# rajabala/Volumetric-Particles-For-Unity

Hardware: AMD Instinct MI355X
Metric: Mvoxels/s filled + Msamples/s raymarched, 32³×32³ grid @1080p (higher is better)
Workload: dtype f32 compute / f16 voxel storage

## Files before the change

### volumetric-particles-for-unity_amd/csrc/api.cpp

```cpp
#include <cmath>
#include <cstdarg>
#include <cstdio>
#include <cstdlib>
#include <cstring>
#include <new>

#include "vpfx_internal.h"

thread_local std::string g_vp_create_error;

int vp_fail(vp_ctx* c, int code, const char* fmt, ...)
{
    char buf[512];
    va_list ap;
    va_start(ap, fmt);
    vsnprintf(buf, sizeof buf, fmt, ap);
    va_end(ap);
    if (c) c->err = buf; else g_vp_create_error = buf;
    return code;
}

namespace {

template <typename T>
// ... 184 lines not shown

VP_EXPORT int vp_abi_version(void) { return VPFX_ABI_VERSION; }

VP_EXPORT const char* vp_last_error(const vp_ctx* c) { return c ? c->err.c_str() : g_vp_create_error.c_str(); }

VP_EXPORT int vp_create(const vp_config* cfg, vp_ctx** out)
{
    if (!cfg || !out) return vp_fail(nullptr, VP_ERR_BAD_ARG, "vp_create: null argument");
    *out = nullptr;
    if (cfg->num_devices < 0 || cfg->num_devices > VP_MAX_LOCAL_DEVICES || cfg->world_size < 0 || cfg->world_size > VP_MAX_RANKS)
        return vp_fail(nullptr, VP_ERR_BAD_ARG, "vp_create: num_devices %d / world_size %d out of range", cfg->num_devices, cfg->world_size);
    if (cfg->num_devices > 1 || cfg->world_size > 1 || (cfg->multi_flags & VP_MULTI_FORCE)) return multi_create(cfg, out);
    if (cfg->num_devices == 1) {
        vp_config one = *cfg;
        one.device = cfg->devices[0];
        return vp_create_single(&one, out);
    }
    return vp_create_single(cfg, out);
}

int vp_create_single(const vp_config* cfg, vp_ctx** out)
{
    vp_ctx* c = nullptr;
    *out = nullptr;
    const int nv = cfg->num_voxels;
    if (cfg->num_mv[0] < 1 || cfg->num_mv[1] < 1 || cfg->num_mv[2] < 1 || !(cfg->mv_scale > 0.f) || cfg->num_border < 0 ||
        2 * cfg->num_border >= nv || cfg->width < 1 || cfg->height < 1)
        return vp_fail(nullptr, VP_ERR_BAD_ARG, "vp_create: bad grid/screen configuration");
    if (nv < 2 || nv > 64)
        return vp_fail(nullptr, VP_ERR_UNSUPPORTED, "vp_create: num_voxels %d outside [2, 64]", nv);
    if ((cfg->reserved[0] != 0 && cfg->reserved[0] != 1) || (cfg->reserved[1] != 0 && cfg->reserved[1] != 1) || cfg->reserved[2] != 0)
        return vp_fail(nullptr, VP_ERR_BAD_ARG, "vp_create: vp_config.reserved = {%d, %d, %d} (0 or the documented switches; an uninitialised struct?)",
                       cfg->reserved[0], cfg->reserved[1], cfg->reserved[2]);
    if ((size_t)cfg->num_mv[0] * cfg->num_mv[1] * cfg->num_mv[2] > ((size_t)1 << 28))
        return vp_fail(nullptr, VP_ERR_UNSUPPORTED, "vp_create: grid too large");
    int z0 = cfg->slab_z0, z1 = cfg->slab_z1;
    if (z0 == 0 && z1 == 0) z1 = cfg->num_mv[2];
    if (z0 < 0 || z1 > cfg->num_mv[2] || z0 >= z1) return vp_fail(nullptr, VP_ERR_BAD_ARG, "vp_create: bad slab [%d,%d)", z0, z1);

    int ndev = 0;
    hipError_t e = hipGetDeviceCount(&ndev);
    if (e != hipSuccess || ndev < 1)
        return vp_fail(nullptr, VP_ERR_NO_DEVICE, "vp_create: no HIP device (%s); libvpfx has no CPU fallback",
                       e != hipSuccess ? hipGetErrorString(e) : "device count 0");
    int dev = cfg->device;
    if (dev < 0) { if (hipGetDevice(&dev) != hipSuccess) dev = 0; }
    if (dev >= ndev) return vp_fail(nullptr, VP_ERR_BAD_ARG, "vp_create: device %d of %d", dev, ndev);

    c = new (std::nothrow) vp_ctx();
    if (!c) return vp_fail(nullptr, VP_ERR_OOM, "vp_create: host allocation failed");
    c->cfg = *cfg;
    c->device = dev;
    if (cfg->multi_flags & VP_MULTI_TEST_HOOKS) { const char* hook = getenv("VPFX_TEST_CHAIN_TIMEOUT"); c->test_chain_timeout = hook && hook[0] == '1'; }
#if VPFX_AB
    { const char* sw = getenv("VPFX_NO_ZPROFILE"); c->no_zprofile = sw && sw[0] == '1'; }
    { const char* sw = getenv("VPFX_RM_FLAT"); c->rm_flat = sw && sw[0] == '1'; }
    { const char* sw = getenv("VPFX_RM_XCD_AFFINE"); c->rm_xcd_affine = sw && sw[0] == '1'; }
#endif
    c->n3 = (size_t)cfg->num_mv[0] * cfg->num_mv[1] * cfg->num_mv[2];
    memset(c->L, 0, sizeof c->L); c->L[0] = c->L[5] = c->L[10] = c->L[15] = 1.f;
    c->h_mvPos = (float*)malloc(c->n3 * 3 * sizeof(float));
    int rc = VP_OK;
    auto fail = [&](int code) { g_vp_create_error = c->err; vp_destroy_single(c); return code; };
    if (!c->h_mvPos) { c->err = "vp_create: host allocation failed"; return fail(VP_ERR_OOM); }
    hl_build_grid(c);
    if ((rc = ensure_device(c))) return fail(rc);
    if (hipDeviceGetAttribute(&c->num_cus, hipDeviceAttributeMultiprocessorCount, dev) != hipSuccess || c->num_cus < 1) c->num_cus = 256;
    const size_t nxy = (size_t)cfg->num_mv[0] * cfg->num_mv[1];
    if ((rc = dev_alloc(c, &c->d_mvPos, c->n3 * 3)) || (rc = dev_alloc(c, &c->d_count, c->n3)) ||
        (rc = dev_alloc(c, &c->d_offsets, c->n3 + 1)) || (rc = dev_alloc(c, &c->d_cursor, c->n3)) ||
        (rc = dev_alloc(c, &c->d_brick_index, c->n3)) || (rc = dev_alloc(c, &c->d_occ_list, c->n3)) ||
        (rc = dev_alloc(c, &c->d_onecol, 2)) || (rc = dev_alloc(c, &c->d_work_counter, 1)) || (rc = dev_alloc(c, &c->d_meta, 1)) ||
        (rc = dev_alloc(c, &c->d_ord, c->n3)) || (rc = dev_alloc(c, &c->d_colcount, nxy)) || (rc = dev_alloc(c, &c->d_chain, lightmap_elems(c))) ||
        (rc = dev_alloc(c, (int4**)&c->d_scan_totals, (c->n3 + 1023) / 1024 + 1)) ||
        (rc = dev_alloc(c, &c->d_lightmap, lightmap_elems(c))) || (rc = dev_alloc(c, &c->d_rank, nxy)) ||
        (rc = dev_alloc(c, &c->d_image, image_elems(c))) || (rc = dev_alloc(c, &c->d_samples, 1)) ||
        (rc = dev_alloc(c, &c->d_zsamples, (size_t)VPFX_ZPROF_COPIES * cfg->num_mv[2])) ||
        (rc = dev_alloc(c, &c->d_tile_order, (size_t)rm_order_ints(rm_num_super_tiles(cfg->width, cfg->height)) + rm_num_super_tiles(cfg->width, cfg->height) + 8)))
        return fail(rc);
#if VPFX_AB
    {
        const int sgx = rm_super_tiles_x(cfg->width), sgy = rm_super_tiles_y(cfg->height), ns = sgx * sgy;
        int side = 1; while (side < sgx || side < sgy) side <<= 1;
        std::vector<int> curve; curve.reserve(ns);
        for (long long d = 0; d < (long long)side * side; ++d) {
            long long tt = d; int x = 0, y = 0;
            for (int sdim = 1; sdim < side; sdim <<= 1) {
                const int rx = 1 & (int)(tt / 2), ry = 1 & ((int)tt ^ rx);
                if (ry == 0) { if (rx == 1) { x = sdim - 1 - x; y = sdim - 1 - y; } const int tmp = x; x = y; y = tmp; }
                x += sdim * rx; y += sdim * ry; tt /= 4;
            }
            if (x < sgx && y < sgy) curve.push_back(y * sgx + x);
        }
        if ((int)curve.size() == ns && (rc = dev_alloc(c, &c->d_tile_curve, (size_t)ns)) == VP_OK) {
            if (hipMemcpy(c->d_tile_curve, curve.data(), (size_t)ns * sizeof(int), hipMemcpyHostToDevice) != hipSuccess) { c->err = "hipMemcpy failed"; return fail(VP_ERR_HIP); }
        } else if (rc) return fail(rc);
    }
#endif
    if (hipHostMalloc((void**)&c->h_meta_host, 2 * sizeof(DevMeta), hipHostMallocMapped | hipHostMallocCoherent) != hipSuccess ||
        hipHostGetDevicePointer((void**)&c->d_meta_host, c->h_meta_host, 0) != hipSuccess) { c->err = "hipHostMalloc failed"; return fail(VP_ERR_HIP); }
    c->h_meta_host[0] = c->h_meta_host[1] = DevMeta{};
    if (hipHostMalloc((void**)&c->h_chain_err, sizeof(int), hipHostMallocMapped) != hipSuccess ||
        hipHostGetDevicePointer((void**)&c->d_chain_err, c->h_chain_err, 0) != hipSuccess) { c->err = "hipHostMalloc failed"; return fail(VP_ERR_HIP); }
    *c->h_chain_err = 0;
    if (hipMemset(c->d_chain, 0, lightmap_elems(c) * sizeof(unsigned long long)) != hipSuccess) { c->err = "hipMemset failed"; return fail(VP_ERR_HIP); }
    for (int s = 0; s < 4; ++s)
        for (int j = 0; j < 2; ++j)
            if (hipEventCreate(&c->ev[s][j]) != hipSuccess) { c->err = "hipEventCreate failed"; return fail(VP_ERR_HIP); }
    *out = c;
    return VP_OK;
}

VP_EXPORT void vp_destroy(vp_ctx* c)
{
    if (!c) return;
    if (c->multi) { multi_destroy(c); return; }
    vp_destroy_single(c);
}

void vp_destroy_single(vp_ctx* c)
{
    if (!c) return;
    (void)hipSetDevice(c->device);
    if (c->stream) (void)hipStreamSynchronize(c->stream); else (void)hipDeviceSynchronize();
    void* dev[] = {c->d_mvPos, c->d_raw, c->d_ws, c->d_rec, c->d_count, c->d_offsets, c->d_cursor, c->d_brick_index,
                   c->d_occ_list, c->d_ids_tmp, c->d_ids, c->d_onecol, c->d_work_counter, c->d_ord, c->d_colcount, c->d_chain, c->d_cube_u8, c->d_meta, c->d_scan_totals, c->d_bricks, c->d_dens_ao,
                   c->d_lightmap, c->d_cubequads, c->d_depthmap, c->d_occluders, c->d_mvtrans, c->d_brick_hit, c->d_rank, c->d_tile_order, c->d_tile_curve, c->d_image, c->d_scene_depth, c->d_samples, c->d_zsamples, c->d_cellinfo, c->d_occmask};
    for (void* p : dev) if (p) (void)hipFree(p);
    mesh_free_all(c);
    device_emitters_orphan_all(c);
    particle_queries_free(c);
    if (c->h_chain_err) (void)hipHostFree(c->h_chain_err);
    if (c->h_meta_host) (void)hipHostFree(c->h_meta_host);
    if (c->copy_stream) { (void)hipStreamSynchronize(c->copy_stream); (void)hipStreamDestroy(c->copy_stream); }
    if (c->ev_image_ready) (void)hipEventDestroy(c->ev_image_ready);
    if (c->ev_image_copied) (void)hipEventDestroy(c->ev_image_copied);
    for (int s = 0; s < 4; ++s) for (int j = 0; j < 2; ++j) if (c->ev[s][j]) (void)hipEventDestroy(c->ev[s][j]);
    free(c->h_mvPos);
    delete c;
}

VP_EXPORT int vp_pin_host_buffer(vp_ctx* c, void* ptr, uint64_t bytes)
{
    if (!c) return VP_ERR_BAD_ARG;
    if (!ptr || !bytes) return vp_fail(c, VP_ERR_BAD_ARG, "vp_pin_host_buffer: null buffer");
    if (c->multi) { VP_HIP(hipHostRegister(ptr, (size_t)bytes, hipHostRegisterPortable)); return VP_OK; }
    int rc = ensure_device(c); if (rc) return rc;
    VP_HIP(hipHostRegister(ptr, (size_t)bytes, hipHostRegisterDefault));
    return VP_OK;
}

VP_EXPORT int vp_unpin_host_buffer(vp_ctx* c, void* ptr)
{
    if (!c) return VP_ERR_BAD_ARG;
    if (!ptr) return vp_fail(c, VP_ERR_BAD_ARG, "vp_unpin_host_buffer: null buffer");
    if (c->multi) { int rcm = multi_sync(c); if (rcm) return rcm; VP_HIP(hipHostUnregister(ptr)); return VP_OK; }
    int rc = ensure_device(c); if (rc) return rc;
    if (c->stream) (void)hipStreamSynchronize(c->stream); else (void)hipDeviceSynchronize();
    if (c->image_copy_pending) { VP_HIP(hipEventSynchronize(c->ev_image_copied)); c->image_copy_pending = false; }
    VP_HIP(hipHostUnregister(ptr));
    return VP_OK;
}

VP_EXPORT int vp_set_stream(vp_ctx* c, void* hip_stream)
{
    if (!c) return VP_ERR_BAD_ARG;
    VP_NO_FANOUT(c, "vp_set_stream (a fan-out context owns one stream per device)");
    c->stream = (hipStream_t)hip_stream;
    return VP_OK;
}

VP_EXPORT int vp_sync(vp_ctx* c)
{
    if (!c) return VP_ERR_BAD_ARG;
    if (c->multi) return multi_sync(c);
    int rc = ensure_device(c); if (rc) return rc;
    { int rcs = stream_sync(c); if (rcs) return rcs; }
    if (c->image_copy_pending) { VP_HIP(hipEventSynchronize(c->ev_image_copied)); c->image_copy_pending = false; }
    return VP_OK;
}
// ... 774 lines not shown
```

### volumetric-particles-for-unity_amd/csrc/raymarch.hip

```cpp
#define VPFX_RM_MAIN_TU 1
#include "raymarch_kernels.h"

namespace {

__device__ __forceinline__ void tile_cost(const RmConsts& k, const int* __restrict__ brick_index, int sgx, float* __restrict__ cost_out, const int sti)
{
    __shared__ float part[4];
    const int wave = threadIdx.x >> 6, lane = threadIdx.x & 63;
    constexpr int SW = 16 << VPFX_RM_LX, SH = 16 << VPFX_RM_LY;
    const float colf = fminf((float)((sti % sgx) * SW + SW / 4 + (SW / 2) * (wave & 1)), (float)k.W - 1.f);
    const float rowf = fminf((float)((sti / sgx) * SH + SH / 4 + (SH / 2) * (wave >> 1)), (float)k.H - 1.f);
    float dx = (2.0f * (colf + 0.5f) / (float)k.W) - 1.0f;
    const float dy = (2.0f * (rowf + 0.5f) / (float)k.H) - 1.0f;
    dx *= k.aspect;
    const float dz = k.neg_inv_tan;
    const float inv = 1.0f / sqrtf((dx * dx + dy * dy) + dz * dz);
    const float dir[3] = {dx * inv, dy * inv, dz * inv};
    const float st = k.zMin / dir[2];
    float o[3], d[3];
#pragma unroll
    for (int r = 0; r < 3; ++r) {
        d[r] = (k.c2g[4 * r] * dir[0] + k.c2g[4 * r + 1] * dir[1]) + k.c2g[4 * r + 2] * dir[2];
        o[r] = d[r] * st + k.c2g[4 * r + 3];
    }
// ... 14 lines not shown
        const int gx = (int)floorf(fmaf(t, d[0], o[0])), gy = (int)floorf(fmaf(t, d[1], o[1])), gz = (int)floorf(fmaf(t, d[2], o[2]));
        const bool occ = gx >= 0 && gx < k.Nx && gy >= 0 && gy < k.Ny && gz >= k.z0 && gz < k.z1 &&
                         brick_index[(gz * k.Ny + gy) * k.Nx + gx] >= 0;
        c = (float)__popcll(__ballot(occ)) * (t1 - t0);
    }
    if (lane == 0) part[wave] = c;
    __syncthreads();
    if (threadIdx.x == 0) cost_out[sti] = (part[0] + part[1]) + (part[2] + part[3]);
}

#define RM_RANK_LDS 4096
#define RM_RANK_COLS 16
__device__ __forceinline__ void column_rank(const RmConsts& k, const float* __restrict__ mvPos, int* __restrict__ rank_out, const int blk)
{
    __shared__ __attribute__((aligned(16))) float keys[RM_RANK_LDS];
    __shared__ int partial[RM_RANK_COLS];
    const int nxy = k.Nx * k.Ny;
    auto key_of = [&](int j) -> float {
        const float dx = mvPos[3 * j] - k.cam_world[0], dy = mvPos[3 * j + 1] - k.cam_world[1], dz = mvPos[3 * j + 2] - k.cam_world[2];
        return (dx * dx + dy * dy) + dz * dz;
    };
    const int i = blk * RM_RANK_COLS + ((int)threadIdx.x & (RM_RANK_COLS - 1)), chunk = (int)threadIdx.x / RM_RANK_COLS;
    if (nxy > RM_RANK_LDS) {
        if (chunk == 0 && i < nxy) {
            const float ki = key_of(i);
            int r = 0;
            for (int j = 0; j < nxy; ++j) { const float kj = key_of(j); r += (kj < ki || (kj == ki && j < i)) ? 1 : 0; }
            rank_out[i] = r;
        }
        return;
    }
    const int npad = (nxy + 3) & ~3;
    for (int j = threadIdx.x; j < npad; j += 256) keys[j] = j < nxy ? key_of(j) : 3.0e38f;
    if (threadIdx.x < RM_RANK_COLS) partial[threadIdx.x] = 0;
    __syncthreads();
    if (i < nxy) {
        constexpr int NCHUNK = 256 / RM_RANK_COLS;
        const int per = ((npad + 4 * NCHUNK - 1) / (4 * NCHUNK)) * 4, j0 = chunk * per, j1 = min(npad, j0 + per);
        const float ki = keys[i];
        int r = 0;
        for (int j = j0; j < j1; j += 4) {
            const float4 kj = *reinterpret_cast<const float4*>(&keys[j]);
            r += (kj.x < ki || (kj.x == ki && j < i)) ? 1 : 0;
            r += (kj.y < ki || (kj.y == ki && j + 1 < i)) ? 1 : 0;
            r += (kj.z < ki || (kj.z == ki && j + 2 < i)) ? 1 : 0;
            r += (kj.w < ki || (kj.w == ki && j + 3 < i)) ? 1 : 0;
        }
        atomicAdd(&partial[threadIdx.x & (RM_RANK_COLS - 1)], r);
    }
    __syncthreads();
    if (chunk == 0 && i < nxy) rank_out[i] = partial[threadIdx.x];
}

__global__ void __launch_bounds__(256)
k_rm_prepare(RmConsts k, const int* __restrict__ brick_index, const float* __restrict__ mvPos, int n3, float4* __restrict__ mvtrans,
             float4* __restrict__ cellinfo , uint32_t* __restrict__ occmask , int* __restrict__ brick_hit,
             unsigned long long* __restrict__ samples, int nprep, int sgx, float* __restrict__ cost_out, int ncost, int* __restrict__ rank_out)
{
    if ((int)blockIdx.x >= nprep + ncost) { column_rank(k, mvPos, rank_out, (int)blockIdx.x - nprep - ncost); return; }
    if ((int)blockIdx.x >= nprep) { tile_cost(k, brick_index, sgx, cost_out, (int)blockIdx.x - nprep); return; }
    const int mi = blockIdx.x * 256 + threadIdx.x;
    if (mi == 0) *samples = 0ull;
    if (mi >= n3) return;
    const int slot = brick_index[mi];
    if (slot >= 0) {
        const float mx = mvPos[3 * mi], my = mvPos[3 * mi + 1], mz = mvPos[3 * mi + 2];
        float tr[3];
#pragma unroll
        for (int r = 0; r < 3; ++r) {
            const float a = k.inv_rows[r * 3], b = k.inv_rows[r * 3 + 1], c = k.inv_rows[r * 3 + 2];
            const float t = -((a * mx + b * my) + c * mz);
            tr[r] = ((a * k.c2w_t[0] + b * k.c2w_t[1]) + c * k.c2w_t[2]) + t * k.c2w_t[3];
        }
        mvtrans[slot] = make_float4(tr[0], tr[1], tr[2], 0.f);
        if (cellinfo) cellinfo[mi] = make_float4(tr[0], tr[1], tr[2], __int_as_float(slot));
        brick_hit[slot] = 0;
    } else if (cellinfo) {
        const float e = __int_as_float(-1);
        cellinfo[mi] = make_float4(e, e, e, e);
    }
    if (occmask && mi % k.Nx == 0) {
        uint32_t word = 0;
        for (int x = 0; x < k.Nx; ++x) word |= (brick_index[mi + x] >= 0 ? 1u : 0u) << x;
        occmask[mi / k.Nx] = word;
    }
}

__global__ void __launch_bounds__(256)
k_order_index(RmConsts k, const int* __restrict__ occ_list, const int* __restrict__ brick_index, const int* __restrict__ rank, int n,
              float4* __restrict__ mvtrans)
{
    const int i = blockIdx.x * 256 + threadIdx.x;
    if (i >= n) return;
    const int nxy = k.Nx * k.Ny, mi = occ_list[i], zz = mi / nxy, cell = mi % nxy;
    const int* occ = brick_index + zz * nxy;
    const int r = rank[cell];
    const bool phaseA = zz <= k.zB;
    int before_in_slice = 0, lower_cells = 0;
    for (int j = 0; j < nxy; ++j) {
        if (occ[j] < 0) continue;
        lower_cells += j < cell ? 1 : 0;
        before_in_slice += (phaseA ? rank[j] > r : rank[j] < r) ? 1 : 0;
    }
    mvtrans[i].w = __int_as_float((i - lower_cells) + before_in_slice);
}

#define MAX_PARTIALS 32
struct BlendArgs { const float4* img[MAX_PARTIALS]; int kind[MAX_PARTIALS]; int n; };

__global__ void __launch_bounds__(256)
k_blend(BlendArgs a, size_t npix, float4* __restrict__ out)
{
    const size_t i = (size_t)blockIdx.x * 256 + threadIdx.x;
    if (i >= npix) return;
    float4 d = make_float4(0.f, 0.f, 0.f, 0.f);
    for (int j = 0; j < a.n; ++j) {
        const float4 s = a.img[j][i];
        if (a.kind[j] == 0) { const float ia = 1.0f - s.w; d.x = s.x + d.x * ia; d.y = s.y + d.y * ia; d.z = s.z + d.z * ia; d.w = s.w + d.w * ia; }
        else { const float ia = 1.0f - d.w; d.x = s.x * ia + d.x; d.y = s.y * ia + d.y; d.z = s.z * ia + d.z; d.w = s.w * ia + d.w; }
    }
    out[i] = d;
}

__global__ void __launch_bounds__(256)
k_composite(const float4* __restrict__ particles, float4* __restrict__ scene, size_t npix)
{
    const size_t i = (size_t)blockIdx.x * 256 + threadIdx.x;
    if (i >= npix) return;
    const float4 s = particles[i];
    float4 d = scene[i];
    const float ia = 1.0f - s.w;
    d.x = s.x + d.x * ia; d.y = s.y + d.y * ia; d.z = s.z + d.z * ia; d.w = s.w + d.w;
    scene[i] = d;
}

}

int launch_raymarch(vp_ctx* c, const RmConsts& k_in, float* d_over, float* d_under, const RmHandoff* handoff)
{
    RmConsts k = k_in;
    k.occ_lds = (VPFX_RM_OCC_LDS && VPFX_RM_CELLINFO && k.Nx <= 32 && k.Nz * k.Ny <= VPFX_RM_OCC_WORDS) ? 1 : 0;
    const RmHandoff ho = (handoff && d_under) ? *handoff : RmHandoff{};
    const int early_out = (c->cfg.no_early_out == 1 || (k.flags & (VP_RM_NO_EARLY_OUT | VP_RM_SHOW_NUM_SAMPLES | VP_RM_SHOW_BLEND_FUNC | VP_RM_SHOW_DRAW_ORDER))) ? 0 : 1;
    k.flags &= ~VP_RM_NO_EARLY_OUT;
    const int nocc = c->h_meta.occupied;
    if ((size_t)nocc > c->mvtrans_cap) {
        if (c->d_mvtrans) VP_HIP(hipFree(c->d_mvtrans));
        c->d_mvtrans = nullptr; c->mvtrans_cap = 0;
        VP_HIP(hipMalloc((void**)&c->d_mvtrans, ((size_t)nocc + nocc / 8 + 16) * sizeof(float4)));
        c->mvtrans_cap = (size_t)nocc + nocc / 8 + 16;
    }
    if ((size_t)nocc > c->brick_hit_cap) {
        if (c->d_brick_hit) VP_HIP(hipFree(c->d_brick_hit));
        c->d_brick_hit = nullptr; c->brick_hit_cap = 0;
        VP_HIP(hipMalloc((void**)&c->d_brick_hit, ((size_t)nocc + nocc / 8 + 16) * sizeof(int)));
        c->brick_hit_cap = (size_t)nocc + nocc / 8 + 16;
    }
#if VPFX_RM_CELLINFO
    if (!c->d_cellinfo) VP_HIP(hipMalloc((void**)&c->d_cellinfo, c->n3 * sizeof(float4)));
    if (k.occ_lds && !c->d_occmask) VP_HIP(hipMalloc((void**)&c->d_occmask, VPFX_RM_OCC_WORDS * sizeof(uint32_t)));
#endif
    c->brick_hit_n = nocc;
    VP_HIP(hipEventRecord(c->ev[2][0], c->stream));
    {
        const int nprep = (int)((c->n3 + 255) / 256), nsuper = rm_num_super_tiles(k.W, k.H);
        const bool ordered = rm_ordered(c, k);
        float* cost = reinterpret_cast<float*>(c->d_tile_order + rm_order_ints(nsuper));
        const int ncost = ordered ? nsuper : 0, nrank = (k.Nx * k.Ny + RM_RANK_COLS - 1) / RM_RANK_COLS;
        hipLaunchKernelGGL(k_rm_prepare, dim3((unsigned)(nprep + ncost + nrank)), dim3(256), 0, c->stream, k, c->d_brick_index, c->d_mvPos,
                           (int)c->n3, c->d_mvtrans, c->d_cellinfo, k.occ_lds ? c->d_occmask : (uint32_t*)nullptr, c->d_brick_hit, c->d_samples,
                           nprep, rm_super_tiles_x(k.W), cost, ncost, c->d_rank);
    }
    if (nocc > 0) {
        if (k.flags & VP_RM_SHOW_DRAW_ORDER)
            hipLaunchKernelGGL(k_order_index, dim3((nocc + 255) / 256), dim3(256), 0, c->stream, k, c->d_occ_list, c->d_brick_index, c->d_rank,
                               nocc, c->d_mvtrans);
    }
    switch (k.nv) {
    case 16: launch_rm_nv<16>(c, k, d_over, d_under, early_out, ho); break;
    case 32: launch_rm_nv<32>(c, k, d_over, d_under, early_out, ho); break;
    case 64: launch_rm_nv<64>(c, k, d_over, d_under, early_out, ho); break;
    default: { int rc = launch_raymarch_generic(c, k, d_over, d_under, early_out, ho); if (rc) return rc; } break;
    }
    VP_HIP(hipGetLastError());
    VP_HIP(hipEventRecord(c->ev[2][1], c->stream));
    c->ev_valid[2] = true;
    return VP_OK;
}

int launch_raymarch_one(vp_ctx* c, const RmConsts& k, int bi, int mi, int blend_over, int order_index, float* d_img)
{
    const float* mp = c->h_mvPos + 3 * (size_t)mi;
    float tr[3];
    for (int r = 0; r < 3; ++r) {
        const float a = k.inv_rows[r * 3], b = k.inv_rows[r * 3 + 1], cc = k.inv_rows[r * 3 + 2];
        const float t = -((a * mp[0] + b * mp[1]) + cc * mp[2]);
        tr[r] = ((a * k.c2w_t[0] + b * k.c2w_t[1]) + cc * k.c2w_t[2]) + t * k.c2w_t[3];
    }
    const float4 trv = make_float4(tr[0], tr[1], tr[2], 0.f);
    const dim3 grid((k.W + 15) / 16, (k.H + 15) / 16), block(256);
    const bool wrap = c->g.b < 1;
    const size_t nv3 = (size_t)k.nv * k.nv * k.nv;
    const uint2* brick = c->d_bricks + (size_t)bi * nv3;
#define VPFX_RM_ONE(NV)                                                                                                        \
    do {                                                                                                                        \
        if (c->bricks_grey) hipLaunchKernelGGL((k_raymarch_one<NV, false, true>), grid, block, 0, c->stream, k, brick, trv,      \
                                     c->d_scene_depth, (float4*)d_img, blend_over, order_index, c->d_samples);                  \
        else if (wrap) hipLaunchKernelGGL((k_raymarch_one<NV, true, false>), grid, block, 0, c->stream, k, brick, trv, c->d_scene_depth,    \
                                     (float4*)d_img, blend_over, order_index, c->d_samples);                                    \
        else      hipLaunchKernelGGL((k_raymarch_one<NV, false, false>), grid, block, 0, c->stream, k, brick, trv, c->d_scene_depth,   \
                                     (float4*)d_img, blend_over, order_index, c->d_samples);                                    \
    } while (0)
    switch (k.nv) {
    case 16: VPFX_RM_ONE(16); break;
    case 32: VPFX_RM_ONE(32); break;
    case 64: VPFX_RM_ONE(64); break;
    default: { int rc = launch_raymarch_one_generic(c, k, brick, tr, blend_over, order_index, d_img); if (rc) return rc; } break;
    }
#undef VPFX_RM_ONE
    VP_HIP(hipGetLastError());
    return VP_OK;
}

int launch_blend(vp_ctx* c, const void* const* d_partials, const int32_t* kinds, int n, float* d_out, size_t npix)
// ... 20 lines not shown
```

### volumetric-particles-for-unity_amd/csrc/raymarch_kernels.h

```cpp
#pragma once
#include <type_traits>

#include "vpfx_internal.h"

namespace {

typedef _Float16 half2_t __attribute__((ext_vector_type(2)));

struct F4 { float x, y, z, w; };

__device__ __forceinline__ F4 unpack_texel(uint2 u)
{
    const half2_t a = __builtin_bit_cast(half2_t, u.x), b = __builtin_bit_cast(half2_t, u.y);
    return F4{(float)a[0], (float)a[1], (float)b[0], (float)b[1]};
}
struct __attribute__((aligned(8))) TexelPair { uint32_t rg0, ba0, rg1, ba1; };

#define VPFX_MIX_FMA(NAME, HI)                                                                                            \
    __device__ __forceinline__ float NAME(float w, uint32_t t, float acc)                                                 \
    {                                                                                                                     \
        float d;                                                                                                          \
        asm("v_fma_mix_f32 %0, %1, %2, %3 op_sel:[0," #HI ",0] op_sel_hi:[0,1,0]" : "=v"(d) : "v"(w), "v"(t), "v"(acc));  \
        return d;                                                                                                         \
    }
// ... 353 lines not shown
    const int t = threadIdx.x;
    for (int i = t; i < 8 * cap; i += 1024) order[i] = -1;
    float acc = 0.f;
    for (int j = t; j < nsuper; j += 1024) { const float c = cost_in[curve[j]]; cost[j] = c; acc += c; }
    part[t] = acc;
    __syncthreads();
    for (int o = 512; o; o >>= 1) { if (t < o) part[t] += part[t + o]; __syncthreads(); }
    const float total = part[0];
    __syncthreads();
    const int per = (nsuper + 1023) / 1024, j0 = min(t * per, nsuper), j1 = min(j0 + per, nsuper);
    const float wc = total > 0.f ? 0.5f / total : 0.f, wn = (total > 0.f ? 0.5f : 1.0f) / (float)nsuper;
    float run = 0.f;
    for (int j = j0; j < j1; ++j) { run += cost[j] * wc + wn; pre[j] = run; }
    part[t] = run;
    __syncthreads();
    if (t == 0) { float a = 0.f; for (int i = 0; i < 1024; ++i) { const float v = part[i]; part[i] = a; a += v; } }
    __syncthreads();
    for (int j = j0; j < j1; ++j) pre[j] += part[t];
    __syncthreads();
    auto region = [&](int j) { return min(7, (int)(8.0f * (j ? pre[j - 1] : 0.f))); };
    if (t < 9) {
        int lo = 0, hi = nsuper;
        while (lo < hi) { const int mid = (lo + hi) >> 1; if (region(mid) >= t) hi = mid; else lo = mid + 1; }
        start[t] = t == 8 ? nsuper : lo;
    }
    __syncthreads();
    for (int j = j0; j < j1; ++j) {
        const int r = region(j), a = start[r], b = start[r + 1];
        const float c = cost[j];
        int rk = 0;
        for (int i = a; i < b; ++i) rk += (cost[i] > c || (cost[i] == c && i < j)) ? 1 : 0;
        if (rk < cap) order[8 * rk + r] = curve[j];
    }
}

#endif

#ifndef VPFX_RM_WAVES
#define VPFX_RM_WAVES 4
#endif
#ifndef VPFX_RM_WAVES_PARTIAL
#define VPFX_RM_WAVES_PARTIAL 3
#endif
#ifndef VPFX_RM_WAVES_GREY
#define VPFX_RM_WAVES_GREY 4
#endif
#define VPFX_RM_HANDOFF_CUTOFF 2.98023224e-8f

template <int NV, bool PARTIAL, bool WRAP, bool FLAGS, bool GREY>
__global__ void __launch_bounds__(64, (PARTIAL && FLAGS) ? VPFX_RM_WAVES_PARTIAL : (GREY && !FLAGS) ? VPFX_RM_WAVES_GREY : VPFX_RM_WAVES)
k_raymarch(RmConsts k, const int* __restrict__ brick_index, const uint2* __restrict__ bricks, const float4* __restrict__ mvtrans,
           const int* __restrict__ rank, const float* __restrict__ scene_depth, float4* __restrict__ img_over, float4* __restrict__ img_under,
           unsigned long long* __restrict__ samples, int* __restrict__ brick_hit, const int* __restrict__ tile_order, int early_out,
           RmHandoff ho, const float4* __restrict__ cellinfo, const uint32_t* __restrict__ occmask, int order_len)
{
    const int lane = threadIdx.x;
    constexpr int LX = VPFX_RM_LX, LY = VPFX_RM_LY, WPS = 4 << (LX + LY);
    constexpr int SW = 16 << LX, SH = 16 << LY;
    const int sgx = (k.W + SW - 1) / SW, sgy = (k.H + SH - 1) / SH;
    const int q = (int)(blockIdx.x >> 3);
    const int within = q % WPS;
    const int slot = (q / WPS) * 8 + (int)(blockIdx.x & 7u);
    if (slot >= (tile_order ? order_len : sgx * sgy)) return;
    const int sti = tile_order ? tile_order[slot] : slot;
    if (sti < 0) return;
    const int bwl = k.lane_transpose ? 6 - k.wave_lx : k.wave_lx, bhl = 6 - bwl;
    const int wx = within & ((SW >> bwl) - 1), wy = within >> (LX + 4 - bwl);
#if VPFX_RM_OCC_LDS
    __shared__ uint32_t s_occ[VPFX_RM_OCC_WORDS];
    if (!FLAGS && k.occ_lds) {
        const int nw = k.Nz * k.Ny;
        for (int i = lane; i < nw; i += 64) s_occ[i] = occmask[i];
        __syncthreads();
    }
#endif
    const int lx = k.lane_transpose ? lane >> bhl : lane & ((1 << bwl) - 1), ly = k.lane_transpose ? lane & ((1 << bhl) - 1) : lane >> bwl;
    const int col = (sti % sgx) * SW + (wx << bwl) + lx;
    const int row = (sti / sgx) * SH + (wy << bhl) + ly;
    if (col >= k.W || row >= k.H) return;

#if VPFX_RM_PROBE == 9
    unsigned long long rm_prof[8] = {};
    const unsigned long long rm_t0 = __builtin_amdgcn_s_memtime();
    unsigned long long rm_last = rm_t0;
#endif
    const RayCtx R = ray_setup(k, col, row, scene_depth);
    VPFX_RM_TICK(0);

    F4 dst{0.f, 0.f, 0.f, 0.f};
    bool storedA = false;
    const size_t pi = (size_t)row * k.W + col;
    int nsamp = 0;

    float tg0, tg1;
    {
        const float bx0 = R.ivx * (0.f - R.ogx), bx1 = R.ivx * ((float)k.Nx - R.ogx);
        const float by0 = R.ivy * (0.f - R.ogy), by1 = R.ivy * ((float)k.Ny - R.ogy);
        const float bz0 = R.ivz * ((float)k.z0 - R.ogz), bz1 = R.ivz * ((float)k.z1 - R.ogz);
        tg0 = fmaxf(fmaxf(fminf(bx0, bx1), fminf(by0, by1)), fminf(bz0, bz1));
        tg1 = fminf(fminf(fmaxf(bx0, bx1), fmaxf(by0, by1)), fmaxf(bz0, bz1));
        if (FLAGS && (k.flags & (VP_RM_SHOW_NUM_SAMPLES | VP_RM_SHOW_BLEND_FUNC | VP_RM_SHOW_DRAW_ORDER))) {
            const float tcs = ((k.camg[0] - R.ogx) * R.dgx + (k.camg[1] - R.ogy) * R.dgy) + (k.camg[2] - R.ogz) * R.dgz;
            tg0 = fmaxf(tg0, tcs);
        } else {
            tg0 = fmaxf(tg0, ((float)R.tCameraG - 2.0f) * k.mvStep);
        }
    }
    const int nxy = k.Nx * k.Ny;
    bool done = !(tg0 <= tg1);
    float tin = 1.0f, aA = 0.f;
    const float cutoff = (PARTIAL && ho.t_in) ? VPFX_RM_HANDOFF_CUTOFF : k.alpha_cutoff;
    if (PARTIAL && ho.t_in) {
        int code = 0;
        for (int j = 0; j < ho.n_in; ++j) code += ho.t_in[(size_t)j * ho.plane + pi];
        tin = __builtin_amdgcn_exp2f(-0.125f * (float)code);
        if (early_out && tin <= cutoff) done = true;
    }

    const int nslab = k.z1 - k.z0;
    const int nA = min(max(k.zB - k.z0 + 1, 0), nslab);
    for (int it = 0; it < nslab && !done; ++it) {
        const int zz = (!FLAGS && it < nA) ? k.z0 + nA - 1 - it : k.z0 + it;
        float ta, tb;
        if (R.dgz != 0.f) {
            const float a = R.ivz * ((float)zz - R.ogz), b = R.ivz * ((float)(zz + 1) - R.ogz);
            ta = fmaxf(fminf(a, b), tg0); tb = fminf(fmaxf(a, b), tg1);
        } else {
            if ((int)floorf(R.ogz) != zz) continue;
            ta = tg0; tb = tg1;
        }
        if (!(ta <= tb)) continue;
        const bool phaseA = zz <= k.zB;
        const bool over = FLAGS && phaseA;
        if (PARTIAL && !phaseA && !storedA) {
            img_over[pi] = make_float4(dst.x, dst.y, dst.z, dst.w);
            aA = dst.w;
            tin *= 1.0f - dst.w;
            dst = F4{0.f, 0.f, 0.f, 0.f};
            storedA = true;
        }
        F4 d = dst;
        const int* occ = brick_index + zz * nxy;
        int last = over ? 0x7fffffff : -1;
        auto walk_start = [&](int& cx, int& cy) { cx = (int)floorf(fmaf(ta, R.dgx, R.ogx)); cy = (int)floorf(fmaf(ta, R.dgy, R.ogy)); };
        int ocx = 0, ocy = 0;
        auto walk_step = [&](int& cx, int& cy, bool& fin) -> int {
            const float tx = R.dgx != 0.f ? R.ivx * ((float)cx + ((R.dgx > 0.f ? 1.0f : 0.0f) - R.ogx)) : 3.0e38f;
            const float ty = R.dgy != 0.f ? R.ivy * ((float)cy + ((R.dgy > 0.f ? 1.0f : 0.0f) - R.ogy)) : 3.0e38f;
            const int cur = (cx >= 0 && cx < k.Nx && cy >= 0 && cy < k.Ny) ? cy * k.Nx + cx : -1;
            ocx = cx; ocy = cy;
            fin = !(fminf(tx, ty) < tb);
            const bool stepx = tx < ty;
            cx += stepx ? (R.dgx > 0.f ? 1 : -1) : 0;
            cy += stepx ? 0 : (R.dgy > 0.f ? 1 : -1);
            return cur;
        };
        const int max_cells = 2 * (k.Nx + k.Ny) + 8;
        bool stream = !over;
        const F4 d_start = d;
        const int ns_start = nsamp;
        int wcx, wcy, walked = 0;
        walk_start(wcx, wcy);
        bool wfin = false;
        for (;;) {
            int best_r = over ? -1 : 0x7fffffff, best_cell = -1;
#if VPFX_RM_CELLINFO
            float4 ci = make_float4(0.f, 0.f, 0.f, __int_as_float(-1));
#endif
            if (stream) {
                while (!wfin && walked < max_cells) {
                    const int cell = walk_step(wcx, wcy, wfin);
                    ++walked;
#if VPFX_RM_CELLINFO
                    if (!FLAGS && cell >= 0) {
#if VPFX_RM_OCC_LDS
                        if (k.occ_lds && !((s_occ[zz * k.Ny + ocy] >> ocx) & 1u)) continue;
#endif
                        const float4 q4 = cellinfo[zz * nxy + cell];
                        const int r = rank[cell];
                        if (__float_as_int(q4.w) >= 0) {
                            if (r > last) { best_r = r; best_cell = cell; ci = q4; }
                            else { d = d_start; nsamp = ns_start; stream = false; last = -1; }
                            break;
                        }
                        continue;
                    }
#endif
                    if (cell >= 0 && occ[cell] >= 0) {
                        const int r = rank[cell];
                        if (r > last) { best_r = r; best_cell = cell; }
                        else { d = d_start; nsamp = ns_start; stream = false; last = -1; }
                        break;
                    }
// ... 388 lines not shown
    VPFX_RM_PROF_DUMMY
    if (!march_mv<NV, WRAP, true, GREY>(k, R, brick, tr, src, nsamp VPFX_RM_PROF_PASS)) return;
    if (k.flags & VP_RM_SHOW_BLEND_FUNC) src = blend_over ? F4{0.5f, 0.5f, 0.f, 1.f} : F4{0.f, 0.5f, 0.5f, 1.f};
    if (k.flags & VP_RM_SHOW_DRAW_ORDER) src = draw_order_color(order_index, k.num_covered);
    const size_t pi = (size_t)row * k.W + col;
    const float4 q = img[pi];
    F4 d{q.x, q.y, q.z, q.w};
    if (blend_over) {
        const float ia = 1.0f - src.w;
        d.x = src.x + d.x * ia; d.y = src.y + d.y * ia; d.z = src.z + d.z * ia; d.w = src.w + d.w * ia;
    } else {
        const float ia = 1.0f - d.w;
        d.x = src.x * ia + d.x; d.y = src.y * ia + d.y; d.z = src.z * ia + d.z; d.w = src.w * ia + d.w;
    }
    if (k.flags & VP_RM_QUANTIZE_UNORM8) { d.x = unorm8(d.x); d.y = unorm8(d.y); d.z = unorm8(d.z); d.w = unorm8(d.w); }
    img[pi] = make_float4(d.x, d.y, d.z, d.w);
    if (nsamp) atomicAdd(samples, (unsigned long long)nsamp);
}

bool rm_ordered(const vp_ctx* c, const RmConsts& k)
{
#ifdef VPFX_RM_NO_ORDER
    return false;
#else
    const int nsuper = rm_num_super_tiles(k.W, k.H);
    const long long waves = (long long)nsuper * (4 << (VPFX_RM_LX + VPFX_RM_LY));
    return nsuper <= RM_ORDER_MAX && waves > (long long)c->num_cus * 8 && k.wave_lx != 4;
#endif
}

template <int NV, bool PARTIAL, bool WRAP, bool FLAGS, bool GREY = false>
void launch_rm_variant(vp_ctx* c, const RmConsts& k, float* d_over, float* d_under, int early_out, const RmHandoff& ho)
{
    const int nsuper = rm_num_super_tiles(k.W, k.H);
    const int* order = nullptr;
    int order_len = nsuper;
#ifndef VPFX_RM_NO_ORDER
    if (rm_ordered(c, k)) {
        float* cost = reinterpret_cast<float*>(c->d_tile_order + rm_order_ints(nsuper));
#if VPFX_AB
        if (c->rm_xcd_affine && c->d_tile_curve) {
            const int cap = rm_order_cap(nsuper);
            hipLaunchKernelGGL(k_tile_regions, dim3(1), dim3(1024), 0, c->stream, cost, c->d_tile_curve, nsuper, cap, c->d_tile_order);
            order_len = 8 * cap;
        } else
#endif
            hipLaunchKernelGGL(k_tile_rank, dim3((nsuper + 63) / 64), dim3(1024), 0, c->stream, cost, nsuper, c->d_tile_order);
        order = c->d_tile_order;
    }
#endif
    const dim3 grid(((order_len + 7) / 8) * 8 * (4 << (VPFX_RM_LX + VPFX_RM_LY))), block(64);
    hipLaunchKernelGGL((k_raymarch<NV, PARTIAL, WRAP, FLAGS, GREY>), grid, block, 0, c->stream, k, c->d_brick_index, c->d_bricks, c->d_mvtrans,
                       c->d_rank, c->d_scene_depth, (float4*)d_over, (float4*)d_under, c->d_samples, c->d_brick_hit, order, early_out, ho,
                       (const float4*)c->d_cellinfo, (const uint32_t*)c->d_occmask, order_len);
}

#if VPFX_AB
template <int NV, bool PARTIAL, bool GREY>
void launch_rm_flat(vp_ctx* c, const RmConsts& k, float* d_over, float* d_under, int early_out, const RmHandoff& ho)
{
    const int nsuper = rm_num_super_tiles(k.W, k.H);
    const int* order = nullptr;
    if (rm_ordered(c, k)) {
        float* cost = reinterpret_cast<float*>(c->d_tile_order + rm_order_ints(nsuper));
        hipLaunchKernelGGL(k_tile_rank, dim3((nsuper + 63) / 64), dim3(1024), 0, c->stream, cost, nsuper, c->d_tile_order);
        order = c->d_tile_order;
    }
    const dim3 grid(((nsuper + 7) / 8) * 8 * (4 << (VPFX_RM_LX + VPFX_RM_LY))), block(64);
    hipLaunchKernelGGL((k_raymarch_flat<NV, PARTIAL, GREY>), grid, block, 0, c->stream, k, c->d_brick_index, c->d_bricks, c->d_mvtrans,
                       c->d_rank, c->d_scene_depth, (float4*)d_over, (float4*)d_under, c->d_samples, c->d_brick_hit, order, early_out, ho);
}

#endif

template <int NV>
void launch_rm_nv(vp_ctx* c, const RmConsts& k, float* d_over, float* d_under, int early_out, const RmHandoff& ho)
{
    const bool wrap = c->g.b < 1;
#if VPFX_AB
    if (c->rm_flat && !wrap && !k.flags) {
        if (c->bricks_grey) { if (d_under) launch_rm_flat<NV, true, true>(c, k, d_over, d_under, early_out, ho); else launch_rm_flat<NV, false, true>(c, k, d_over, d_under, early_out, ho); }
        else { if (d_under) launch_rm_flat<NV, true, false>(c, k, d_over, d_under, early_out, ho); else launch_rm_flat<NV, false, false>(c, k, d_over, d_under, early_out, ho); }
        return;
    }
#endif
    const int sel = (d_under ? 4 : 0) | (wrap ? 2 : 0) | (k.flags ? 1 : 0);
    if (c->bricks_grey) {
        switch (sel & 5) {
        case 0: launch_rm_variant<NV, false, false, false, true>(c, k, d_over, d_under, early_out, ho); break;
        case 1: launch_rm_variant<NV, false, false, true, true>(c, k, d_over, d_under, early_out, ho); break;
        case 4: launch_rm_variant<NV, true, false, false, true>(c, k, d_over, d_under, early_out, ho); break;
        default: launch_rm_variant<NV, true, false, true, true>(c, k, d_over, d_under, early_out, ho); break;
        }
        return;
    }
    switch (sel) {
    case 0: launch_rm_variant<NV, false, false, false>(c, k, d_over, d_under, early_out, ho); break;
    case 1: launch_rm_variant<NV, false, false, true>(c, k, d_over, d_under, early_out, ho); break;
    case 2: launch_rm_variant<NV, false, true, false>(c, k, d_over, d_under, early_out, ho); break;
    case 3: launch_rm_variant<NV, false, true, true>(c, k, d_over, d_under, early_out, ho); break;
    case 4: launch_rm_variant<NV, true, false, false>(c, k, d_over, d_under, early_out, ho); break;
    case 5: launch_rm_variant<NV, true, false, true>(c, k, d_over, d_under, early_out, ho); break;
    case 6: launch_rm_variant<NV, true, true, false>(c, k, d_over, d_under, early_out, ho); break;
    default: launch_rm_variant<NV, true, true, true>(c, k, d_over, d_under, early_out, ho); break;
    }
}

// ... 2 lines not shown
```

### volumetric-particles-for-unity_amd/csrc/vpfx_internal.h

```cpp
#pragma once

#include <hip/hip_runtime.h>
#include <stdint.h>
#include <string>
#include <vector>

#include "../../include/vpfx.h"

#define VP_EXPORT extern "C" __attribute__((visibility("default")))

#define VPFX_CFG_NO_LDS_CUBEMAP 1
#define VPFX_CFG_NO_GREY_BRICKS 1

struct MeshShape { int64_t first_vertex, n_vertices, first_triangle, n_triangles; };
struct MeshInstDev {
    float m[12];
    int32_t first_triangle, n_triangles;
    int32_t mirrored, pad;
};
struct MeshTri { float4 p0, p1, p2; };

struct GridConsts {
    int Nx, Ny, Nz, nv, b, z0, z1, pad0;
    float s, sb, one, inv_sb;
    float Linv[12];
    float lsO[3];
    float Rl[9];
    float Rsb[9];
    float rowsb[9];
    float fwd[3];
    float gc[3];
};

struct PsysConsts {
    float L2W[12];
    float axis[3];
    int   rot_in_radians;
};

struct FillConsts {
    float opacity_factor, D, one_minus_D, init_light;
    float amb[3];
    int   fade;
    float bq, inv_a;
    float camp[3];
    float dstep[3];
    int   cubeS;
    float half_s, half_s_m05;
    int   border_index;
    float D_over_255;
    int   lds_pitch;
    int   d_is_one;
    int   grey;
};

struct RmConsts {
    int W, H, Nx, Ny, Nz, nv, z0, z1;
    int zB, steps, soft, partial;
    int wave_lx;
    int flags, num_covered, lane_transpose, occ_lds;
    float aspect, neg_inv_tan, zMin, s;
    float mvStep, inv_mvStep, nearc, farc;
    float c2m_lin[9];
    float inv_rows[9];
    float c2w_t[4];
    float c2g[12];
    float camg[3];
    float cam_world[3];
    float texScale, texBias;
    float inv_soft;
    float alpha_cutoff;
};

#ifndef VPFX_ZPROF_COPIES
#define VPFX_ZPROF_COPIES 64
#endif
struct RmHandoff {
    const uint8_t* t_in; int n_in; size_t plane;
    uint8_t* t_out0; uint8_t* t_out1;
    unsigned* zsamples;
};

struct DevMeta {
    int occupied;
    int pairs;
    int max_pairs;
    int unsorted_lists;
};

struct vp_multi;

struct vp_ctx {
    vp_config cfg{};
    vp_multi* multi = nullptr;
    bool test_chain_timeout = false;
    bool rm_xcd_affine = false;
    int* d_tile_curve = nullptr;
    bool rm_flat = false;
    bool no_zprofile = false;
    int device = 0;
    hipStream_t stream = nullptr;
    hipStream_t copy_stream = nullptr;
    hipEvent_t ev_image_ready = nullptr, ev_image_copied = nullptr;
    bool image_copy_pending = false;
    GridConsts g{};
    bool have_frame = false, have_particles = false, binned = false, filled = false, local_done = false, fill_begun = false;

    float L[16]{}, gc[3]{};
    float* h_mvPos = nullptr;
    float* d_mvPos = nullptr;

    int P = 0, P_cap = 0;
    size_t raw_cap = 0;
    uint8_t* d_raw = nullptr;
    float4* d_ws = nullptr;
    float* d_rec = nullptr;
    vp_particle_layout lay{};
    PsysConsts psys{};

    size_t n3 = 0;
    int* d_count = nullptr;
    int* d_offsets = nullptr;
    int* d_cursor = nullptr;
    int* d_brick_index = nullptr;
    int* d_occ_list = nullptr;
// ... 9 lines not shown
    int bin_seq = 0;

    uint2* d_bricks = nullptr;
    bool bricks_grey = false;
    size_t brick_cap = 0;
    float2* d_dens_ao = nullptr;
    size_t dens_cap = 0;
    float* d_lightmap = nullptr;
    float4* d_cubequads = nullptr;
    int cubeS = 0;
    uint32_t* d_cube_u8 = nullptr;
    size_t cube_u8_cap = 0;
    int cube_u8_S = 0;
    int* d_work_counter = nullptr;
    int* d_ord = nullptr;
    int* d_colcount = nullptr;
    unsigned long long* d_chain = nullptr;
    uint32_t chain_seq = 0;
    int* h_chain_err = nullptr;
    int* d_chain_err = nullptr;
    int num_cus = 0;
    float* d_depthmap = nullptr;
    bool have_depthmap = false;
    FillConsts fc{};
    const float* finish_tau_all = nullptr;
    int finish_n_before = 0;

    vp_occluder* d_occluders = nullptr;
    int n_occluders = 0, occluders_cap = 0;
    unsigned occl_gen = 1, frame_gen = 1;
    unsigned eye_depth_gen = 0; vp_camera eye_depth_cam{};
    unsigned light_depth_gen = 0, light_depth_frame = 0; float light_depth_planes[3] = {0.f, 0.f, 0.f};
    float* d_mesh_pos = nullptr;
    int32_t* d_mesh_idx = nullptr;
    std::vector<MeshShape> mesh_shapes;
    MeshInstDev* d_mesh_inst = nullptr;
    uint32_t* d_mesh_inst_first = nullptr;
    int n_mesh_inst = 0, n_mesh_inst_placed = 0;
    uint32_t n_mesh_tris = 0;
    MeshTri* d_mesh_rec = nullptr; size_t mesh_rec_cap = 0;
    uint32_t* d_mesh_tile_count = nullptr; unsigned long long* d_mesh_tile_start = nullptr; size_t mesh_tiles_cap = 0;
    uint32_t* d_mesh_list = nullptr; size_t mesh_list_cap = 0;
    unsigned long long* h_mesh_total = nullptr;

    std::vector<vp_device_emitter*> emitters;

    uint32_t* d_query = nullptr;
    uint32_t* h_query = nullptr;
    int* d_cover = nullptr;
    size_t cover_cap = 0;

    float4* d_mvtrans = nullptr;
    size_t mvtrans_cap = 0;
    uint32_t* d_occmask = nullptr;
    float4* d_cellinfo = nullptr;
    int* d_rank = nullptr;
    int* d_tile_order = nullptr;
    float* d_image = nullptr;
    float* d_scene_depth = nullptr;
    unsigned long long* d_samples = nullptr;
    unsigned* d_zsamples = nullptr;
    int* d_brick_hit = nullptr;
    size_t brick_hit_cap = 0;
    int brick_hit_n = 0;
    long long last_samples = 0;

    hipEvent_t ev[4][2]{};
    bool ev_valid[4] = {false, false, false, false};

    std::string err;
};

extern thread_local std::string g_vp_create_error;

int vp_fail(vp_ctx* c, int code, const char* fmt, ...);

#define VP_HIP(call)                                                                                  \
    do {                                                                                              \
        hipError_t e_ = (call);                                                                       \
        if (e_ != hipSuccess)                                                                         \
            return vp_fail(c, e_ == hipErrorOutOfMemory ? VP_ERR_OOM : VP_ERR_HIP, "%s failed: %s (%s:%d)", \
                           #call, hipGetErrorString(e_), __FILE__, __LINE__);                         \
    } while (0)

void   hl_build_grid(vp_ctx* c);
void   hl_build_psys(vp_ctx* c, const float m[16]);
void   hl_build_fill_consts(vp_ctx* c, const vp_fill_params* p);
int    hl_z_boundary(const vp_ctx* c, const vp_camera* cam);
#ifndef VPFX_AB
#define VPFX_AB 0
#endif
#ifndef VPFX_RM_LX
#define VPFX_RM_LX 2
#endif
#ifndef VPFX_RM_LY
#define VPFX_RM_LY 1
#endif
inline int rm_super_tiles_x(int W) { return (((W + 15) / 16) + (1 << VPFX_RM_LX) - 1) >> VPFX_RM_LX; }
inline int rm_super_tiles_y(int H) { return (((H + 15) / 16) + (1 << VPFX_RM_LY) - 1) >> VPFX_RM_LY; }
inline int rm_num_super_tiles(int W, int H) { return rm_super_tiles_x(W) * rm_super_tiles_y(H); }
inline int rm_order_cap(int nsuper) { return nsuper / 4 + 2; }
inline int rm_order_ints(int nsuper) { return 8 * rm_order_cap(nsuper) + 8; }
void   hl_plan_slabs(int nz, int world, const double* fill_ms, const double* rm_ms, int rm_groups, int* cuts );
int    hl_blend_plan(int world, const int* cuts, int zb, int* chain, int* plan_rank, int* plan_which, int* plan_kind, int* straddler);
int    hl_exchange_plan(int world, int rank, int strad, int all_gather, int phase, vp_xop* ops, int cap);
void   hl_chain_groups(int world, int rm_groups, int* group_of_pos );
// ... 64 lines not shown
```

Measured before the change: 170,700.

## Skip empty z-slabs in raymarch using per-slab occupied bounding rectangles

Adds a prepare-stage block per z slab that reduces the occupied brick columns to an xy bounding rectangle packed into one word. The raymarch kernel loads these rectangles into LDS and skips a slab when the ray segment's xy extent falls outside the padded rectangle. This avoids per-cell occupancy lookups for empty regions. The cost is extra prepare blocks, LDS use and a per-slab test. It is enabled by a heuristic (wave count above eight per CU) and can be overridden with an environment variable.

Measured after the change: 172,500 (median of 6 runs). 1.01x the previous value.

```diff
diff --git a/volumetric-particles-for-unity_amd/csrc/api.cpp b/volumetric-particles-for-unity_amd/csrc/api.cpp
--- a/volumetric-particles-for-unity_amd/csrc/api.cpp
+++ b/volumetric-particles-for-unity_amd/csrc/api.cpp
@@ -260,6 +260,7 @@
     c->cfg = *cfg;
     c->device = dev;
     if (cfg->multi_flags & VP_MULTI_TEST_HOOKS) { const char* hook = getenv("VPFX_TEST_CHAIN_TIMEOUT"); c->test_chain_timeout = hook && hook[0] == '1'; }
+    { const char* sw = getenv("VPFX_RM_NO_SPACE_SKIP"); c->rm_space_skip = !sw ? 0 : sw[0] == '1' ? -1 : sw[0] == '0' ? 1 : 0; }
 #if VPFX_AB
     { const char* sw = getenv("VPFX_NO_ZPROFILE"); c->no_zprofile = sw && sw[0] == '1'; }
     { const char* sw = getenv("VPFX_RM_FLAT"); c->rm_flat = sw && sw[0] == '1'; }
@@ -333,7 +334,7 @@
     if (c->stream) (void)hipStreamSynchronize(c->stream); else (void)hipDeviceSynchronize();
     void* dev[] = {c->d_mvPos, c->d_raw, c->d_ws, c->d_rec, c->d_count, c->d_offsets, c->d_cursor, c->d_brick_index,
                    c->d_occ_list, c->d_ids_tmp, c->d_ids, c->d_onecol, c->d_work_counter, c->d_ord, c->d_colcount, c->d_chain, c->d_cube_u8, c->d_meta, c->d_scan_totals, c->d_bricks, c->d_dens_ao,
-                   c->d_lightmap, c->d_cubequads, c->d_depthmap, c->d_occluders, c->d_mvtrans, c->d_brick_hit, c->d_rank, c->d_tile_order, c->d_tile_curve, c->d_image, c->d_scene_depth, c->d_samples, c->d_zsamples, c->d_cellinfo, c->d_occmask};
+                   c->d_lightmap, c->d_cubequads, c->d_depthmap, c->d_occluders, c->d_mvtrans, c->d_brick_hit, c->d_rank, c->d_tile_order, c->d_tile_curve, c->d_image, c->d_scene_depth, c->d_samples, c->d_zsamples, c->d_cellinfo, c->d_occmask, c->d_slab_rect};
     for (void* p : dev) if (p) (void)hipFree(p);
     mesh_free_all(c);
     device_emitters_orphan_all(c);
diff --git a/volumetric-particles-for-unity_amd/csrc/raymarch.hip b/volumetric-particles-for-unity_amd/csrc/raymarch.hip
--- a/volumetric-particles-for-unity_amd/csrc/raymarch.hip
+++ b/volumetric-particles-for-unity_amd/csrc/raymarch.hip
@@ -90,11 +90,38 @@
     if (chunk == 0 && i < nxy) rank_out[i] = partial[threadIdx.x];
 }
 
+__device__ __forceinline__ void slab_rect(const RmConsts& k, const int* __restrict__ brick_index, uint32_t* __restrict__ out, const int zz)
+{
+    __shared__ int part[4][4];
+    const int nxy = k.Nx * k.Ny, wave = threadIdx.x >> 6, lane = threadIdx.x & 63;
+    int x0 = 31, x1 = 0, y0 = 2047, y1 = 0;
+    if (zz >= k.z0 && zz < k.z1) {
+        const int* occ = brick_index + (size_t)zz * nxy;
+        for (int c = threadIdx.x; c < nxy; c += 256)
+            if (occ[c] >= 0) {
+                const int y = c / k.Nx, x = c - y * k.Nx;
+                x0 = min(x0, x); x1 = max(x1, x); y0 = min(y0, y); y1 = max(y1, y);
+            }
+    }
+    for (int o = 32; o; o >>= 1) {
+        x0 = min(x0, __shfl_xor(x0, o)); x1 = max(x1, __shfl_xor(x1, o));
+        y0 = min(y0, __shfl_xor(y0, o)); y1 = max(y1, __shfl_xor(y1, o));
+    }
+    if (lane == 0) { part[wave][0] = x0; part[wave][1] = x1; part[wave][2] = y0; part[wave][3] = y1; }
+    __syncthreads();
+    if (threadIdx.x == 0) {
+        for (int w = 1; w < 4; ++w) { x0 = min(x0, part[w][0]); x1 = max(x1, part[w][1]); y0 = min(y0, part[w][2]); y1 = max(y1, part[w][3]); }
+        out[zz] = (uint32_t)x0 | (uint32_t)x1 << 5 | (uint32_t)y0 << 10 | (uint32_t)y1 << 21;
+    }
+}
+
 __global__ void __launch_bounds__(256)
 k_rm_prepare(RmConsts k, const int* __restrict__ brick_index, const float* __restrict__ mvPos, int n3, float4* __restrict__ mvtrans,
              float4* __restrict__ cellinfo , uint32_t* __restrict__ occmask , int* __restrict__ brick_hit,
-             unsigned long long* __restrict__ samples, int nprep, int sgx, float* __restrict__ cost_out, int ncost, int* __restrict__ rank_out)
-{
+             unsigned long long* __restrict__ samples, int nprep, int sgx, float* __restrict__ cost_out, int ncost, int* __restrict__ rank_out,
+             int nrank, uint32_t* __restrict__ rect_out)
+{
+    if ((int)blockIdx.x >= nprep + ncost + nrank) { slab_rect(k, brick_index, rect_out, (int)blockIdx.x - nprep - ncost - nrank); return; }
     if ((int)blockIdx.x >= nprep + ncost) { column_rank(k, mvPos, rank_out, (int)blockIdx.x - nprep - ncost); return; }
     if ((int)blockIdx.x >= nprep) { tile_cost(k, brick_index, sgx, cost_out, (int)blockIdx.x - nprep); return; }
     const int mi = blockIdx.x * 256 + threadIdx.x;
@@ -178,6 +205,10 @@
 {
     RmConsts k = k_in;
     k.occ_lds = (VPFX_RM_OCC_LDS && VPFX_RM_CELLINFO && k.Nx <= 32 && k.Nz * k.Ny <= VPFX_RM_OCC_WORDS) ? 1 : 0;
+    const long long waves = (long long)rm_num_super_tiles(k.W, k.H) * (4 << (VPFX_RM_LX + VPFX_RM_LY));
+    const bool skip = k.occ_lds && k.Nz <= VPFX_RM_SKIP_RECTS && !(k.flags & ~VP_RM_NO_EARLY_OUT) &&
+                      (c->rm_space_skip > 0 || (c->rm_space_skip == 0 && waves > (long long)c->num_cus * 8));
+    if (skip) k.occ_lds |= 2;
     const RmHandoff ho = (handoff && d_under) ? *handoff : RmHandoff{};
     const int early_out = (c->cfg.no_early_out == 1 || (k.flags & (VP_RM_NO_EARLY_OUT | VP_RM_SHOW_NUM_SAMPLES | VP_RM_SHOW_BLEND_FUNC | VP_RM_SHOW_DRAW_ORDER))) ? 0 : 1;
     k.flags &= ~VP_RM_NO_EARLY_OUT;
@@ -197,6 +228,7 @@
 #if VPFX_RM_CELLINFO
     if (!c->d_cellinfo) VP_HIP(hipMalloc((void**)&c->d_cellinfo, c->n3 * sizeof(float4)));
     if (k.occ_lds && !c->d_occmask) VP_HIP(hipMalloc((void**)&c->d_occmask, VPFX_RM_OCC_WORDS * sizeof(uint32_t)));
+    if (skip && !c->d_slab_rect) VP_HIP(hipMalloc((void**)&c->d_slab_rect, VPFX_RM_SKIP_RECTS * sizeof(uint32_t)));
 #endif
     c->brick_hit_n = nocc;
     VP_HIP(hipEventRecord(c->ev[2][0], c->stream));
@@ -205,9 +237,9 @@
         const bool ordered = rm_ordered(c, k);
         float* cost = reinterpret_cast<float*>(c->d_tile_order + rm_order_ints(nsuper));
         const int ncost = ordered ? nsuper : 0, nrank = (k.Nx * k.Ny + RM_RANK_COLS - 1) / RM_RANK_COLS;
-        hipLaunchKernelGGL(k_rm_prepare, dim3((unsigned)(nprep + ncost + nrank)), dim3(256), 0, c->stream, k, c->d_brick_index, c->d_mvPos,
+        hipLaunchKernelGGL(k_rm_prepare, dim3((unsigned)(nprep + ncost + nrank + (skip ? k.Nz : 0))), dim3(256), 0, c->stream, k, c->d_brick_index, c->d_mvPos,
                            (int)c->n3, c->d_mvtrans, c->d_cellinfo, k.occ_lds ? c->d_occmask : (uint32_t*)nullptr, c->d_brick_hit, c->d_samples,
-                           nprep, rm_super_tiles_x(k.W), cost, ncost, c->d_rank);
+                           nprep, rm_super_tiles_x(k.W), cost, ncost, c->d_rank, nrank, c->d_slab_rect);
     }
     if (nocc > 0) {
         if (k.flags & VP_RM_SHOW_DRAW_ORDER)
diff --git a/volumetric-particles-for-unity_amd/csrc/raymarch_kernels.h b/volumetric-particles-for-unity_amd/csrc/raymarch_kernels.h
--- a/volumetric-particles-for-unity_amd/csrc/raymarch_kernels.h
+++ b/volumetric-particles-for-unity_amd/csrc/raymarch_kernels.h
@@ -429,7 +429,8 @@
 k_raymarch(RmConsts k, const int* __restrict__ brick_index, const uint2* __restrict__ bricks, const float4* __restrict__ mvtrans,
            const int* __restrict__ rank, const float* __restrict__ scene_depth, float4* __restrict__ img_over, float4* __restrict__ img_under,
            unsigned long long* __restrict__ samples, int* __restrict__ brick_hit, const int* __restrict__ tile_order, int early_out,
-           RmHandoff ho, const float4* __restrict__ cellinfo, const uint32_t* __restrict__ occmask, int order_len)
+           RmHandoff ho, const float4* __restrict__ cellinfo, const uint32_t* __restrict__ occmask, int order_len,
+           const uint32_t* __restrict__ slab_rect)
 {
     const int lane = threadIdx.x;
     constexpr int LX = VPFX_RM_LX, LY = VPFX_RM_LY, WPS = 4 << (LX + LY);
@@ -445,9 +446,15 @@
     const int wx = within & ((SW >> bwl) - 1), wy = within >> (LX + 4 - bwl);
 #if VPFX_RM_OCC_LDS
     __shared__ uint32_t s_occ[VPFX_RM_OCC_WORDS];
+    __shared__ float4 s_rect[VPFX_RM_SKIP_RECTS];
     if (!FLAGS && k.occ_lds) {
         const int nw = k.Nz * k.Ny;
         for (int i = lane; i < nw; i += 64) s_occ[i] = occmask[i];
+        if ((k.occ_lds & 2) && lane < k.Nz) {
+            const uint32_t r = slab_rect[lane];
+            s_rect[lane] = make_float4((float)((int)(r & 31u) - 1), (float)((int)((r >> 5) & 31u) + 2), (float)((int)((r >> 10) & 2047u) - 1),
+                                       (float)((int)(r >> 21) + 2));
+        }
         __syncthreads();
     }
 #endif
@@ -516,6 +523,13 @@
             dst = F4{0.f, 0.f, 0.f, 0.f};
             storedA = true;
         }
+#if VPFX_RM_OCC_LDS
+        if (!FLAGS && (k.occ_lds & 2)) {
+            const float4 rc = s_rect[zz];
+            const float xa = fmaf(ta, R.dgx, R.ogx), xb = fmaf(tb, R.dgx, R.ogx), ya = fmaf(ta, R.dgy, R.ogy), yb = fmaf(tb, R.dgy, R.ogy);
+            if (fmaxf(xa, xb) < rc.x || fminf(xa, xb) >= rc.y || fmaxf(ya, yb) < rc.z || fminf(ya, yb) >= rc.w) continue;
+        }
+#endif
         F4 d = dst;
         const int* occ = brick_index + zz * nxy;
         int last = over ? 0x7fffffff : -1;
@@ -1010,7 +1024,7 @@
     const dim3 grid(((order_len + 7) / 8) * 8 * (4 << (VPFX_RM_LX + VPFX_RM_LY))), block(64);
     hipLaunchKernelGGL((k_raymarch<NV, PARTIAL, WRAP, FLAGS, GREY>), grid, block, 0, c->stream, k, c->d_brick_index, c->d_bricks, c->d_mvtrans,
                        c->d_rank, c->d_scene_depth, (float4*)d_over, (float4*)d_under, c->d_samples, c->d_brick_hit, order, early_out, ho,
-                       (const float4*)c->d_cellinfo, (const uint32_t*)c->d_occmask, order_len);
+                       (const float4*)c->d_cellinfo, (const uint32_t*)c->d_occmask, order_len, (const uint32_t*)c->d_slab_rect);
 }
 
 #if VPFX_AB
diff --git a/volumetric-particles-for-unity_amd/csrc/vpfx_internal.h b/volumetric-particles-for-unity_amd/csrc/vpfx_internal.h
--- a/volumetric-particles-for-unity_amd/csrc/vpfx_internal.h
+++ b/volumetric-particles-for-unity_amd/csrc/vpfx_internal.h
@@ -71,6 +71,7 @@
     float inv_soft;
     float alpha_cutoff;
 };
+#define VPFX_RM_SKIP_RECTS 64
 
 #ifndef VPFX_ZPROF_COPIES
 #define VPFX_ZPROF_COPIES 64
@@ -186,6 +187,8 @@
 
     float4* d_mvtrans = nullptr;
     size_t mvtrans_cap = 0;
+    int rm_space_skip = 0;
+    uint32_t* d_slab_rect = nullptr;
     uint32_t* d_occmask = nullptr;
     float4* d_cellinfo = nullptr;
     int* d_rank = nullptr;
```
